# wangtong627/COR

Hardware: AMD Instinct MI355X
Metric: query triplets/sec (forward + similarity + top-k) (higher is better)
Workload: dtype bf16

## Files before the change

cor_amd/_native.py:

```python
from __future__ import annotations

import ctypes as C
import os

_HERE = os.path.dirname(os.path.abspath(__file__))
LIB_PATH = os.environ.get("COR_AMD_LIB") or os.path.join(_HERE, "csrc", "libcor_amd.so")

F32, BF16, F16, BF16X3 = 0, 1, 2, 3
ACT_NONE, ACT_GELU_ERF, ACT_RELU, ACT_SIGMOID, ACT_GELU_TANH = 0, 1, 2, 3, 4
EINVAL, ENOSUPPORT = -1, -2
TOPK_FORCE_LISTS, TOPK_NO_FALLBACK, TOPK_FORCE_GLOBAL_THRESHOLD, TOPK_WAVE_FINAL = 1, 2, 8, 16
TOPK_KMAX = 256
FILTER_EQ, FILTER_NE = 0, 1
MERGE_NMAX = 4096
ORDER_REVERSE = 1 << 30
KERNEL_ROWLANE, KERNEL_FEWQ, KERNEL_FLASH_MFMA, KERNEL_FLASH_PIPELINED, KERNEL_WINDOW_BLOCK = 1, 2, 3, 4, 5
import numpy as _np
Q_PRESCALE_HD64 = float(_np.float32(0.125) * _np.float32(1.4426950408889634))

_p, _i, _l, _f, _ll = C.c_void_p, C.c_int, C.c_long, C.c_float, C.c_longlong

SIGNATURES = {
    "cor_version": [],
    "cor_gemm": [_p, _l, _p, _l, _i, _p, _l, _i, _i, _i, _i, _p, _i, _p, _p, _l, _i, _i, _p],
    "cor_layernorm": [_p, _i, _p, _i, _p, _p, _i, _i, _f, _i, _p],
    "cor_attention": [_p, _l, _l, _p, _l, _l, _p, _l, _l, _i, _p, _l, _l, _i, _i, _i, _i, _i, _i, _f, _p],
    "cor_attention_f32": [_p, _l, _l, _p, _l, _l, _p, _l, _l, _p, _l, _l, _i, _i, _i, _i, _i, _i, _f, _p],
    "cor_attention_kernel_id": [_i, _i, _i, _i, _i, _i],
    "cor_sam_attention": [_p, _i, _p, _i, _p, _p, _p, _i, _i, _i, _i, _i, _f, _i, _p],
    "cor_patchify": [_p, _p, _i, _i, _i, _i, _i, _i, _i, _p],
    "cor_im2col3x3": [_p, _i, _p, _i, _i, _i, _i, _p],
    "cor_add": [_p, _i, _p, _i, _p, _i, _l, _l, _p],
    "cor_copy_rows": [_p, _l, _i, _p, _l, _i, _i, _i, _p],
    "cor_split_x3": [_p, _l, _p, _l, _l, _i, _i, _p],
    "cor_tokens_to_nchw": [_p, _i, _p, _i, _i, _i, _p],
    "cor_nchw_to_tokens": [_p, _p, _i, _i, _i, _i, _p],
    "cor_l2norm_rows": [_p, _i, _p, _i, _i, _i, _f, _p],
    "cor_embed_tokens": [_p, _p, _p, _p, _i, _i, _i, _i, _p],
    "cor_bilinear": [_p, _p, _i, _i, _i, _i, _i, _i, _p],
    "cor_conv3x3s2_small": [_p, _i, _p, _p, _p, _i, _i, _i, _i, _i, _p],
    "cor_dwconv7x7": [_p, _p, _p, _p, _i, _i, _i, _i, _i, _p],
    "cor_adapter_pool": [_p, _p, _p, _i, _i, _i, _i, _p],
    "cor_masked_pool": [_p, _i, _p, _p, _i, _i, _i, _i, _i, _p],
    "cor_region_pool": [_p, _p, _p, _p, _i, _i, _i, _i, _i, _i, _i, _p],
    "cor_fuse_gate": [_p, _p, _p, _p, _p, _i, _i, _p],
    "cor_fuse_mix": [_p, _p, _p, _i, _i, _p],
    "cor_dense_pe": [_p, _p, _i, _i, _p],
    "cor_upscale_shuffle": [_p, _i, _p, _p, _p, _f, _i, _p, _i, _i, _i, _i, _i, _p],
# ... 63 lines not shown
```

cor_amd/csrc/flash_attn.hip:

```cpp
#include <cstdlib>
#include <type_traits>

#include "common.h"

typedef short s16x4 __attribute__((ext_vector_type(4)));

namespace {

struct FlashArgs {
  const bf16_t* q; const bf16_t* k; const bf16_t* v; void* o;
  long q_sb, q_st, k_sb, k_st, v_sb, v_st, o_sb, o_st;
  int H, Tq, Tk;
  float scale_log2;
  float tbl_scale;
  const bf16_t* pad_row; const float* rel_h; const float* rel_w;
  int grid, S, nW, d3;
  int nqt;
  int rev;
};

constexpr int KT = 64;
constexpr int TILE_B = KT * 128;
constexpr int KV_BYTES = 4 * TILE_B;
constexpr int AUX_PER_WAVE = 8192;
constexpr float LOG2E = 1.4426950408889634f;

__device__ __forceinline__ int acc_row(int e, int h) { return (e & 3) + 8 * (e >> 2) + 4 * h; }

__device__ __forceinline__ float other_half(float x) {
  const unsigned u = __float_as_uint(x);
  const auto r = __builtin_amdgcn_permlane32_swap(u, u, false, false);
  return __uint_as_float((threadIdx.x & 32) ? r[0] : r[1]);
}

typedef float f32x2_t __attribute__((ext_vector_type(2)));
typedef __bf16 bf16x2_t __attribute__((ext_vector_type(2)));
__device__ __forceinline__ uint32_t pk2(float a, float b) {
  const f32x2_t v = {a, b};
  return __builtin_bit_cast(uint32_t, __builtin_convertvector(v, bf16x2_t));
}
__device__ __forceinline__ uint4 pack8(float f0, float f1, float f2, float f3, float f4, float f5, float f6, float f7) {
  uint4 u;
  u.x = pk2(f0, f1); u.y = pk2(f2, f3); u.z = pk2(f4, f5); u.w = pk2(f6, f7);
  return u;
}

__device__ __forceinline__ float sum2_bf16(uint32_t pair, float acc) {
  return __builtin_amdgcn_fdot2_f32_bf16(__builtin_bit_cast(bf16x2_t, pair), __builtin_bit_cast(bf16x2_t, 0x3f803f80u), acc, false);
}
__device__ __forceinline__ float max3f_(float a, float b, float c) { return fmaxf(fmaxf(a, b), c); }

__device__ __forceinline__ uint4 table_frag(const float* tbl, int j, int c, int h) {
  const float* p = tbl + (long)j * 64 + 16 * c + 8 * h;
  const f32x4 a = *(const f32x4*)p, b = *(const f32x4*)(p + 4);
  return pack8(a[0], a[1], a[2], a[3], b[0], b[1], b[2], b[3]);
}

template <typename TO, int HD, typename OFF>
__device__ __forceinline__ void store_o_rows(const f32x16 (&o)[(HD + 31) / 32], float inv, char* stg, TO* out, int lane, OFF&& off) {
  constexpr int DB = (HD + 31) / 32;
  const int r = lane & 31, h = lane >> 5;
  if constexpr (sizeof(TO) == 2) {
    constexpr int SR = HD * 2 + 16, NCHO = HD * 2 / 16;
#pragma unroll
    for (int db = 0; db < DB; ++db)
#pragma unroll
      for (int g = 0; g < 4; ++g) {
        if (db * 32 + 8 * g + 8 <= HD) {
          uint2 u;
          u.x = pk2(o[db][4 * g] * inv, o[db][4 * g + 1] * inv); u.y = pk2(o[db][4 * g + 2] * inv, o[db][4 * g + 3] * inv);
          *(uint2*)(stg + r * SR + (db * 32 + 8 * g + 4 * h) * 2) = u;
        }
      }
    __builtin_amdgcn_fence(__ATOMIC_ACQ_REL, "wavefront");
#pragma unroll
    for (int i = 0; i < (32 * NCHO + 63) / 64; ++i) {
      const int idx = lane + 64 * i, j = idx / NCHO, ch = idx - j * NCHO;
      if (idx < 32 * NCHO) {
        const uint4 v = *(const uint4*)(stg + j * SR + ch * 16);
        const long e = off(j);
        if (e >= 0) *(uint4*)(out + e + ch * 8) = v;
      }
    }
// ... 929 lines not shown
    }
  }
  {
    asm volatile("s_waitcnt vmcnt(0)" ::: "memory");
    const char* Vs = Vring + ((nt - 1) & 3) * TILE_B;
#pragma unroll
    for (int kb = 0; kb < 2; ++kb)
#pragma unroll
      for (int ks = 0; ks < 2; ++ks)
#pragma unroll
        for (int db = 0; db < 2; ++db) {
          const char* vb = Vs + (kb * 32 + ks * 16) * 128 + v_trd[db];
          const s16x4 v0 = __builtin_amdgcn_ds_read_tr16_b64_v4i16((__attribute__((address_space(3))) s16x4*)(vb));
          const s16x4 v1 = __builtin_amdgcn_ds_read_tr16_b64_v4i16((__attribute__((address_space(3))) s16x4*)(vb + 8 * 128));
          const u32x4 vfr = __builtin_bit_cast(u32x4, __builtin_shufflevector(v0, v1, 0, 1, 2, 3, 4, 5, 6, 7));
#pragma unroll
          for (int qb = 0; qb < 2; ++qb)
            asm volatile("v_mfma_f32_32x32x16_bf16 %0, %1, %2, %0" : "+a"(o[qb][db]) : "a"(vfr), "v"(pf[qb][kb][ks]));
        }
    asm volatile("s_nop 7\n\ts_nop 7\n\ts_nop 7\n\ts_nop 7" ::: "memory");
  }
#pragma unroll
  for (int qb = 0; qb < 2; ++qb) {
    const float l = lsum[qb][0] + lsum[qb][1];
    const float inv = 1.0f / (l + other_half(l));
    auto off = [&](int j) -> long { return ((long)b * g2 + qh * S + qb * 32 + j) * (long)(a.H * 64) + head * 64; };
    store_o_rows<TO, 64>(o[qb], inv, (char*)aux, (TO*)a.o, lane, off);
    __builtin_amdgcn_fence(__ATOMIC_ACQ_REL, "wavefront");
  }
}

constexpr int WIN_ROWS = 224, WIN_KV = WIN_ROWS * 128, WIN_T = 27 * 32 * 4, WIN_LDS = 2 * WIN_KV + 7 * WIN_T;

template <typename TO>
__global__ void __launch_bounds__(448, 4) win_attn(const FlashArgs a) {
  extern __shared__ __attribute__((aligned(16))) char smem[];
  const int tid = threadIdx.x, lane = tid & 63, wave = __builtin_amdgcn_readfirstlane(tid >> 6);
  const int r = lane & 31, h = lane >> 5;
  const int bid = a.rev ? (int)gridDim.x - 1 - (int)blockIdx.x : (int)blockIdx.x;
  const int head = bid % a.H, win = bid / a.H;
  const int nw2 = a.nW * a.nW, b = win / nw2, wi = win - b * nw2, wy = wi / a.nW, wx = wi - wy * a.nW;
  const int g2 = a.grid * a.grid;
  char* Kt = smem; char* Vt = smem + WIN_KV;
  float* T = (float*)(smem + 2 * WIN_KV + wave * WIN_T);

  {
    const unsigned lds0 = __builtin_amdgcn_readfirstlane((unsigned)(size_t)((__attribute__((address_space(3))) char*)smem));
    const int sl = lane & 7;
    long colp[2]; bool okx[2];
#pragma unroll
    for (int hf = 0; hf < 2; ++hf) {
      const int kw = min(8 * hf + (lane >> 3), 13), x = wx * 14 + kw;
      okx[hf] = x < a.grid;
      colp[hf] = ((long)b * g2 + x) * a.d3 + head * 64;
    }
#pragma unroll
    for (int i8 = 0; i8 < 8; ++i8) {
      const int i = wave * 8 + i8;
      const bool isv = i >= 28;
      const int ii = isv ? i - 28 : i, kh = ii >> 1, hf = ii & 1, y = wy * 14 + kh;
      const int chunk = isv ? (sl ^ (((lane >> 4) & 1) << 2)) : (sl ^ (4 * hf + (lane >> 4)));
      const long plane = (long)(isv ? 2 : 1) * a.H * 64 + chunk * 8;
      const bf16_t* src = (y < a.grid && okx[hf]) ? a.q + colp[hf] + (long)y * a.grid * a.d3 + plane : a.pad_row + head * 64 + plane;
      glds16(src, lds0 + (isv ? WIN_KV : 0) + ii * 1024);
    }
  }

  const int tq = min(wave * 32 + r, 195);
  const int qh = (tq * 4682) >> 16, qw = tq - 14 * qh;
  uint4 qf[4];
  {
    const int y = wy * 14 + qh, x = wx * 14 + qw;
    const bf16_t* qp = (y < a.grid && x < a.grid) ? a.q + ((long)b * g2 + (long)y * a.grid + x) * a.d3 + head * 64 : a.pad_row + head * 64;
#pragma unroll
    for (int c = 0; c < 4; ++c) qf[c] = *(const uint4*)(qp + 16 * c + 8 * h);
  }

  float colb[8];
  uint4 tf[2][4];
#pragma unroll
  for (int tbl = 0; tbl < 2; ++tbl)
#pragma unroll
    for (int c = 0; c < 4; ++c) tf[tbl][c] = table_frag(tbl == 0 ? a.rel_w : a.rel_h, min(r, 26), c, h);
#pragma unroll
  for (int tbl = 0; tbl < 2; ++tbl) {
    f32x16 acc;
#pragma unroll
    for (int e = 0; e < 16; ++e) acc[e] = 0.f;
#pragma unroll
    for (int c = 0; c < 4; ++c)
      acc = __builtin_amdgcn_mfma_f32_32x32x16_bf16(__builtin_bit_cast(bf16x8, tf[tbl][c]), __builtin_bit_cast(bf16x8, qf[c]), acc, 0, 0, 0);
#pragma unroll
    for (int e = 0; e < 16; ++e) {
      const int row = acc_row(e, h);
      if (row < 27) T[row * 32 + r] = acc[e] * a.tbl_scale;
    }
    __builtin_amdgcn_fence(__ATOMIC_ACQ_REL, "wavefront");
    if (tbl == 0) {
#pragma unroll
      for (int e8 = 0; e8 < 8; ++e8) {
        const int kw = (e8 & 3) + 8 * (e8 >> 2) + 4 * h;
        colb[e8] = kw < 14 ? T[(qw - min(kw, 13) + 13) * 32 + r] : -INFINITY;
      }
      __builtin_amdgcn_fence(__ATOMIC_ACQ_REL, "wavefront");
    }
  }

  if (a.scale_log2 != 1.0f) {
#pragma unroll
    for (int c = 0; c < 4; ++c) {
      uint32_t w[4] = {qf[c].x, qf[c].y, qf[c].z, qf[c].w};
#pragma unroll
      for (int i = 0; i < 4; ++i) w[i] = pk2(__uint_as_float(w[i] << 16) * a.scale_log2, __uint_as_float(w[i] & 0xffff0000u) * a.scale_log2);
      qf[c] = make_uint4(w[0], w[1], w[2], w[3]);
    }
  }

  asm volatile("s_waitcnt vmcnt(0)" ::: "memory");
  __syncthreads();

  const int sw = (r >> 1) & 7;
  const int k_rd = r * 128, v_tr = (4 * h + ((lane & 15) >> 2)) * 128 + (16 * ((lane >> 4) & 1) + 4 * (lane & 3)) * 2;
  const int v_trd[2] = {v_tr + ((lane >> 3) & 1) * 64, v_tr + (1 - ((lane >> 3) & 1)) * 64};
  const int t_rd = (qh + 13) * 32 + r;
  f32x16 o[2], lsum;
#pragma unroll
  for (int e = 0; e < 16; ++e) { o[0][e] = 0.f; o[1][e] = 0.f; lsum[e] = 0.f; }
  float m = 0.f;
  const uint4 ones = make_uint4(0x3F803F80u, 0x3F803F80u, 0x3F803F80u, 0x3F803F80u);
#pragma unroll
  for (int blk = 0; blk < 7; ++blk) {
    const char* Kb = Kt + blk * 32 * 128 + k_rd;
    uint4 kf[4];
#pragma unroll
    for (int c = 0; c < 4; ++c) kf[c] = *(const uint4*)(Kb + (((2 * c + h) ^ sw) << 4));
    const float rm0 = T[t_rd - 32 * (2 * blk)] - m, rm1 = T[t_rd - 32 * (2 * blk + 1)] - m;
    f32x16 s;
#pragma unroll
    for (int e = 0; e < 16; ++e) s[e] = colb[e & 7] + (e < 8 ? rm0 : rm1);
#pragma unroll
    for (int c = 0; c < 4; ++c)
      s = __builtin_amdgcn_mfma_f32_32x32x16_bf16(__builtin_bit_cast(bf16x8, kf[c]), __builtin_bit_cast(bf16x8, qf[c]), s, 0, 0, 0);
    float mloc = max3f_(max3f_(s[0], s[1], s[2]), max3f_(s[3], s[4], s[5]), max3f_(s[6], s[7], s[8]));
    mloc = fmaxf(max3f_(mloc, max3f_(s[9], s[10], s[11]), max3f_(s[12], s[13], s[14])), s[15]);
    mloc = fmaxf(mloc, other_half(mloc));
    if (blk == 0 || __builtin_amdgcn_ballot_w64(mloc > 8.0f) != 0) {
      const float d = blk == 0 ? mloc : fmaxf(mloc, 0.f);
      const float alpha = __builtin_amdgcn_exp2f(-d);
      m += d;
#pragma unroll
      for (int e = 0; e < 16; ++e) s[e] -= d;
      if (blk != 0) {
        lsum[1] *= alpha; lsum[2] *= alpha;
#pragma unroll
        for (int e = 0; e < 16; ++e) { o[0][e] *= alpha; o[1][e] *= alpha; }
      }
    }
    uint4 pf[2];
    {
      f32x16 p;
#pragma unroll
      for (int e = 0; e < 16; ++e) p[e] = __builtin_amdgcn_exp2f(s[e]);
      pf[0] = pack8(p[0], p[1], p[2], p[3], p[4], p[5], p[6], p[7]);
      pf[1] = pack8(p[8], p[9], p[10], p[11], p[12], p[13], p[14], p[15]);
      lsum[1] = sum2_bf16(pf[0].y, sum2_bf16(pf[0].x, lsum[1])); lsum[2] = sum2_bf16(pf[0].w, sum2_bf16(pf[0].z, lsum[2]));
      lsum[1] = sum2_bf16(pf[1].y, sum2_bf16(pf[1].x, lsum[1])); lsum[2] = sum2_bf16(pf[1].w, sum2_bf16(pf[1].z, lsum[2]));
    }
#pragma unroll
    for (int ks = 0; ks < 2; ++ks) {
#pragma unroll
      for (int db = 0; db < 2; ++db) {
        const char* vb = Vt + (blk * 32 + ks * 16) * 128 + v_trd[db];
        const s16x4 v0 = __builtin_amdgcn_ds_read_tr16_b64_v4i16((__attribute__((address_space(3))) s16x4*)(vb));
        const s16x4 v1 = __builtin_amdgcn_ds_read_tr16_b64_v4i16((__attribute__((address_space(3))) s16x4*)(vb + 8 * 128));
        const uint2 u0 = __builtin_bit_cast(uint2, v0), u1 = __builtin_bit_cast(uint2, v1);
        const uint4 vfr = make_uint4(u0.x, u0.y, u1.x, u1.y);
        o[db] = __builtin_amdgcn_mfma_f32_32x32x16_bf16(__builtin_bit_cast(bf16x8, vfr), __builtin_bit_cast(bf16x8, pf[ks]), o[db], 0, 0, 0);
      }
    }
  }

  const float lhalf = lsum[1] + lsum[2];
  const float inv = 1.0f / (lhalf + other_half(lhalf));
  char* stg = (char*)T;
  TO* out = (TO*)a.o;
  auto off = [&](int jq) -> long {
    const int tj = wave * 32 + jq;
    if (tj >= 196) return -1;
    const int jh = (tj * 4682) >> 16, y = wy * 14 + jh, x = wx * 14 + (tj - 14 * jh);
    if (y >= a.grid || x >= a.grid) return -1;
    return ((long)b * g2 + (long)y * a.grid + x) * (long)(a.H * 64) + head * 64;
  };
  const long e0 = off(lane >> 2), e1 = off((lane >> 2) + 16);
  const int rd0 = (lane >> 2) * 80 + (lane & 3) * 16;
  __builtin_amdgcn_fence(__ATOMIC_ACQ_REL, "wavefront");
  if constexpr (sizeof(TO) == 2) {
#pragma unroll
    for (int db = 0; db < 2; ++db) {
#pragma unroll
      for (int g = 0; g < 4; ++g) {
        uint2 u;
        u.x = pk2(o[db][4 * g] * inv, o[db][4 * g + 1] * inv); u.y = pk2(o[db][4 * g + 2] * inv, o[db][4 * g + 3] * inv);
        *(uint2*)(stg + r * 80 + (8 * g + 4 * h) * 2) = u;
      }
      __builtin_amdgcn_fence(__ATOMIC_ACQ_REL, "wavefront");
      const uint4 v0 = *(const uint4*)(stg + rd0), v1 = *(const uint4*)(stg + rd0 + 16 * 80);
      if (e0 >= 0) *(uint4*)(out + e0 + db * 32 + (lane & 3) * 8) = v0;
      if (e1 >= 0) *(uint4*)(out + e1 + db * 32 + (lane & 3) * 8) = v1;
      __builtin_amdgcn_fence(__ATOMIC_ACQ_REL, "wavefront");
    }
  } else {
#pragma unroll
    for (int qd = 0; qd < 4; ++qd) {
      const int db = qd >> 1, g0 = 2 * (qd & 1);
#pragma unroll
      for (int gg = 0; gg < 2; ++gg) {
        const int g = g0 + gg;
        const f32x4 v4 = {o[db][4 * g] * inv, o[db][4 * g + 1] * inv, o[db][4 * g + 2] * inv, o[db][4 * g + 3] * inv};
        *(f32x4*)(stg + r * 80 + (8 * gg + 4 * h) * 4) = v4;
      }
      __builtin_amdgcn_fence(__ATOMIC_ACQ_REL, "wavefront");
      const f32x4 v0 = *(const f32x4*)(stg + rd0), v1 = *(const f32x4*)(stg + rd0 + 16 * 80);
      if (e0 >= 0) *(f32x4*)(out + e0 + qd * 16 + (lane & 3) * 4) = v0;
      if (e1 >= 0) *(f32x4*)(out + e1 + qd * 16 + (lane & 3) * 4) = v1;
      __builtin_amdgcn_fence(__ATOMIC_ACQ_REL, "wavefront");
    }
  }
}

template <typename TO>
int launch_win(const FlashArgs& a, int nwin, hipStream_t s) {
  static DevOnce once;
  cor_max_dyn_lds((const void*)win_attn<TO>, WIN_LDS, once);
  hipLaunchKernelGGL((win_attn<TO>), dim3(nwin * a.H), dim3(448), WIN_LDS, s, a);
  COR_CHECK_LAUNCH();
  return 0;
}

template <typename TO, bool STAMP = false, bool CB = false>
int launch_global_pipe(const FlashArgs& a, int nb, hipStream_t s) {
  const size_t lds = 6 * TILE_B + 4 * AUX_PER_WAVE;
  static DevOnce once;
  cor_max_dyn_lds((const void*)flash_global_pipe<TO, STAMP, CB>, (int)lds, once);
  FlashArgs b = a;
  b.nqt = cdiv(a.Tq, 128);
  hipLaunchKernelGGL((flash_global_pipe<TO, STAMP, CB>), dim3(b.nqt * a.H * nb), dim3(256), lds, s, b);
  COR_CHECK_LAUNCH();
  return 0;
}

template <typename TO, int DBG = 0>
int launch_global_w64(const FlashArgs& a, int nb, hipStream_t s) {
  const size_t lds = 8 * TILE_B + 4 * 64 * 64 * 4;
  static DevOnce once;
  cor_max_dyn_lds((const void*)flash_global_w64<TO, DBG>, (int)lds, once);
  FlashArgs b = a;
  b.nqt = a.Tq / 256;
  hipLaunchKernelGGL((flash_global_w64<TO, DBG>), dim3(b.nqt * a.H * nb), dim3(256), lds, s, b);
  COR_CHECK_LAUNCH();
  return 0;
}

template <int MODE, typename TO, int HD = 64>
int launch(const FlashArgs& a, int nb, hipStream_t s) {
  constexpr int ROWB = HD == 64 ? 128 : 208;
  const size_t lds = 4 * KT * ROWB + (MODE == 0 ? 0 : 4 * AUX_PER_WAVE);
  static DevOnce once;
// ... 2 lines not shown
  b.nqt = cdiv(a.Tq, 128);
  hipLaunchKernelGGL((flash_fwd<MODE, TO, HD>), dim3(b.nqt * a.H * nb), dim3(256), lds, s, b);
  COR_CHECK_LAUNCH();
  return 0;
}
template <int MODE, int HD>
int launch_t(const FlashArgs& a, int nb, int out_dtype, hipStream_t s) {
  if (out_dtype == COR_BF16) return launch<MODE, bf16_t, HD>(a, nb, s);
  if (out_dtype == COR_F32) return launch<MODE, float, HD>(a, nb, s);
  return COR_ENOSUPPORT;
}

}

int cor_flash_plain_bf16(const void* q, long q_sb, long q_st, const void* k, long k_sb, long k_st, const void* v, long v_sb, long v_st,
                         void* out, long o_sb, long o_st, int out_dtype, int B, int H, int Tq, int Tk, int hd, float scale, hipStream_t s) {
  if ((q_st | k_st | v_st | q_sb | k_sb | v_sb) & 7) return COR_ENOSUPPORT;
  if (((uintptr_t)q | (uintptr_t)k | (uintptr_t)v | (uintptr_t)out) & 15) return COR_ENOSUPPORT;
  if ((o_st | o_sb) & 7) return COR_ENOSUPPORT;
  FlashArgs a{};
  a.q = (const bf16_t*)q; a.k = (const bf16_t*)k; a.v = (const bf16_t*)v; a.o = out;
  a.q_sb = q_sb; a.q_st = q_st; a.k_sb = k_sb; a.k_st = k_st; a.v_sb = v_sb; a.v_st = v_st; a.o_sb = o_sb; a.o_st = o_st;
  a.H = H; a.Tq = Tq; a.Tk = Tk; a.scale_log2 = scale * LOG2E; a.tbl_scale = LOG2E; a.S = 1; a.grid = 1; a.nW = 1;
  if (hd == 64) return launch_t<0, 64>(a, B, out_dtype, s);
  if (hd == 72) return launch_t<0, 72>(a, B, out_dtype, s);
  if (hd == 80) return launch_t<0, 80>(a, B, out_dtype, s);
  return COR_ENOSUPPORT;
}

int cor_flash_sam_bf16(const void* qkv, void* out, int out_dtype, const void* pad_row, const float* rel_h, const float* rel_w, int B,
                       int H, int hd, int grid, int window, float q_prescale, int variant, hipStream_t s) {
  if (hd != 64 && hd != 80) return COR_ENOSUPPORT;
  const int rev = (variant & COR_ORDER_REVERSE) ? 1 : 0;
  variant &= ~COR_ORDER_REVERSE;
#ifdef COR_PROBES
  if (variant != 0 && variant != 1 && variant != 2 && variant != 4 && variant != 9 && !(variant >= 16 && variant < 4096)) return COR_EINVAL;
#else
  if (variant != 0 && variant != 1 && variant != 2 && variant != 4) return COR_EINVAL;
#endif
  if (((uintptr_t)qkv & 15) || ((uintptr_t)out & 15) || ((uintptr_t)rel_h & 15) || ((uintptr_t)rel_w & 15)) return COR_ENOSUPPORT;
  FlashArgs a{};
  a.q = (const bf16_t*)qkv; a.o = out; a.H = H; a.rev = rev;
  a.scale_log2 = LOG2E / sqrtf((float)hd) / q_prescale; a.tbl_scale = LOG2E / q_prescale;
  if (hd == 64 && fabsf(a.scale_log2 - 1.0f) < 1e-6f) { a.scale_log2 = 1.0f; a.tbl_scale = 8.0f; }
  a.pad_row = (const bf16_t*)pad_row; a.rel_h = rel_h; a.rel_w = rel_w; a.grid = grid; a.d3 = 3 * H * hd;
  if (window == 0) {
    if (grid != 64) return COR_ENOSUPPORT;
    a.S = 64; a.Tq = a.Tk = grid * grid; a.nW = 1;
#ifdef COR_PROBES
    if (const char* e = getenv("COR_ATTN_TK")) a.Tk = atoi(e);
#endif
    if (hd == 80) return launch_t<1, 80>(a, B, out_dtype, s);
#ifdef COR_PROBES
    if (variant >= 16 && out_dtype == COR_BF16 && a.scale_log2 == 1.0f) {
      switch (variant - 16) {
        case 1: return launch_global_w64<bf16_t, 1>(a, B, s);
        case 2: return launch_global_w64<bf16_t, 2>(a, B, s);
        case 3: return launch_global_w64<bf16_t, 3>(a, B, s);
        case 4: return launch_global_w64<bf16_t, 4>(a, B, s);
        case 8: return launch_global_w64<bf16_t, 8>(a, B, s);
        case 16: return launch_global_w64<bf16_t, 16>(a, B, s);
        case 32: return launch_global_w64<bf16_t, 32>(a, B, s);
        case 64: return launch_global_w64<bf16_t, 64>(a, B, s);
        case 96: return launch_global_w64<bf16_t, 96>(a, B, s);
        case 7: return launch_global_w64<bf16_t, 7>(a, B, s);
        case 127: return launch_global_w64<bf16_t, 127>(a, B, s);
        case 128: return launch_global_w64<bf16_t, 128>(a, B, s);
        case 256: return launch_global_w64<bf16_t, 256>(a, B, s);
        case 384: return launch_global_w64<bf16_t, 384>(a, B, s);
        case 512: return launch_global_w64<bf16_t, 512>(a, B, s);
        default: return COR_EINVAL;
      }
    }
    if (variant == 9) {
      if (out_dtype == COR_BF16) return launch_global_pipe<bf16_t, true>(a, B, s);
      if (out_dtype == COR_F32) return launch_global_pipe<float, true>(a, B, s);
    }
#endif
    if (variant == 4 && a.scale_log2 == 1.0f) {
      if (out_dtype == COR_BF16) return launch_global_w64<bf16_t>(a, B, s);
      if (out_dtype == COR_F32) return launch_global_w64<float>(a, B, s);
    }
    if (variant == 0 && a.scale_log2 == 1.0f) {
      if (out_dtype == COR_BF16) return launch_global_pipe<bf16_t, false, true>(a, B, s);
      if (out_dtype == COR_F32) return launch_global_pipe<float, false, true>(a, B, s);
    }
    if (variant == 0 || variant == 2 || variant == 4) {
      if (out_dtype == COR_BF16) return launch_global_pipe<bf16_t>(a, B, s);
      if (out_dtype == COR_F32) return launch_global_pipe<float>(a, B, s);
    }
    if (out_dtype == COR_BF16) return launch<1, bf16_t>(a, B, s);
    if (out_dtype == COR_F32) return launch<1, float>(a, B, s);
    return COR_ENOSUPPORT;
  }
  if (window != 14 || ((uintptr_t)pad_row & 15)) return COR_ENOSUPPORT;
  a.S = 14; a.Tq = a.Tk = 196; a.nW = (grid + 13) / 14;
  if (hd == 80) return launch_t<2, 80>(a, B * a.nW * a.nW, out_dtype, s);
  if (variant != 1) {
    if (out_dtype == COR_BF16) return launch_win<bf16_t>(a, B * a.nW * a.nW, s);
    if (out_dtype == COR_F32) return launch_win<float>(a, B * a.nW * a.nW, s);
    return COR_ENOSUPPORT;
  }
  if (out_dtype == COR_BF16) return launch<2, bf16_t>(a, B * a.nW * a.nW, s);
  if (out_dtype == COR_F32) return launch<2, float>(a, B * a.nW * a.nW, s);
  return COR_ENOSUPPORT;
}
```

cor_amd/engine.py:

```python
from __future__ import annotations

import math

import torch

from . import _native as nat
from . import ops
from .ops import ACT_NONE, ACT_GELU_ERF, ACT_RELU, ACT_SIGMOID, ACT_GELU_TANH, X3

F32 = torch.float32


def _round_up(x, m):
    return (x + m - 1) // m * m


class _Packer:

    def __init__(self, sd: dict, T: torch.dtype):
        dev = next(iter(sd.values())).device
        if dev.type != "cuda":
            raise RuntimeError("cor_amd: the model must live on a GPU (model.to('cuda')); there is no CPU path")
        self.sd, self.T, self.W = sd, T, {}

# ... 7 lines not shown
    def lin(self, p):
        self.mat(p + "weight")
        self.f32(p + "bias")

    def ln(self, p):
        self.f32(p + "weight")
        self.f32(p + "bias")

    def patch_embed(self, p, dim, patch):
        kp = 3 * patch * patch
        K = _round_up(kp, 16)
        self.W[p + "patch.K"] = K
        w = self.sd[p + "patch_embed.proj.weight"].detach().reshape(dim, kp)
        if K != kp:
            w = torch.nn.functional.pad(w, (0, K - kp))
        self.mat(p + "patch_embed.proj.weight", w)
        self.f32(p + "patch_embed.proj.bias")
        self.f32(p + "pos_embed", self.sd[p + "pos_embed"].detach().reshape(-1, dim))


def pack_sam_encoder(pk: _Packer, cfg: dict, p="image_encoder."):
    sd, W, d = pk.sd, pk.W, cfg["dim"]
    pk.patch_embed(p, d, cfg["patch"])
    for i in range(cfg["depth"]):
        b = f"{p}blocks.{i}."
        pk.ln(b + "norm1."); pk.ln(b + "norm2.")
        qs = nat.Q_PRESCALE_HD64 if (pk.T == torch.bfloat16 and d // cfg["heads"] == 64) else 1.0
        W[b + "attn.q_prescale"] = qs
        wq, bq = sd[b + "attn.qkv.weight"].detach().to(F32).clone(), sd[b + "attn.qkv.bias"].detach().to(F32).clone()
        wq[:d] *= qs; bq[:d] *= qs
        pk.mat(b + "attn.qkv.weight", wq); pk.f32(b + "attn.qkv.bias", bq)
        pk.lin(b + "attn.proj."); pk.lin(b + "mlp.lin1."); pk.lin(b + "mlp.lin2.")
        pk.f32(b + "attn.rel_pos_h"); pk.f32(b + "attn.rel_pos_w")
        pk.mat(b + "attn.pad_row", bq)
    pk.mat(p + "neck.0.weight", sd[p + "neck.0.weight"].detach().reshape(cfg["out"], d))
    pk.ln(p + "neck.1."); pk.ln(p + "neck.3.")
    w3 = sd[p + "neck.2.weight"].detach()
    pk.mat(p + "neck.2.weight", w3.permute(0, 2, 3, 1).reshape(w3.shape[0], -1))


def pack_prompt_encoder(pk: _Packer, p="prompt_encoder.", size=64):
    g = pk.sd[p + "pe_layer.positional_encoding_gaussian_matrix"].detach().to(F32).contiguous()
    pk.W["prompt.dense_pe"] = ops.dense_pe(g, size)
    pk.f32("prompt.no_mask", pk.sd[p + "no_mask_embed.weight"].detach().reshape(-1))


def pack_siglip(pk: _Packer, g: dict, p="support_branch.siglip.model."):
    v = p + "visual.trunk."
    pk.patch_embed(v, g["dim"], g["patch"])
    for i in range(g["depth"]):
        b = f"{v}blocks.{i}."
        pk.ln(b + "norm1."); pk.ln(b + "norm2.")
        pk.lin(b + "attn.qkv."); pk.lin(b + "attn.proj."); pk.lin(b + "mlp.fc1."); pk.lin(b + "mlp.fc2.")
    pk.ln(v + "norm.")
    t = p + "text."
    pk.f32(t + "token_embedding.weight"); pk.f32(t + "positional_embedding")
    for i in range(g["t_depth"]):
        b = f"{t}transformer.resblocks.{i}."
        pk.ln(b + "ln_1."); pk.ln(b + "ln_2.")
        pk.mat(b + "attn.in_proj_weight"); pk.f32(b + "attn.in_proj_bias")
        pk.lin(b + "attn.out_proj."); pk.lin(b + "mlp.c_fc."); pk.lin(b + "mlp.c_proj.")
    pk.ln(t + "ln_final."); pk.lin(t + "text_projection.")


def pack_mask_adapter(pk: _Packer, m="support_branch.mask_pooling."):
    sd = pk.sd
# ... 71 lines not shown
    pack_support_head(pkq, mask_pooling)
    pack_mask_decoder(pk)
    if pkq is not pk:
        pk.W.update(pkq.W)
    return pk.W


def _lin(W, p, a, out_dtype, act=ACT_NONE, residual=None, col_scale=None, out=None, reverse=False, x3=False):
    return ops.gemm(a, W[p + "weight"], out_dtype=out_dtype, bias=W[p + "bias"], act=act, residual=residual,
                    col_scale=col_scale, out=out, reverse=reverse, x3=x3)


def _ln(W, p, x, eps, out_dtype, act=ACT_NONE, reverse=False):
    return ops.layernorm(x, W[p + "weight"], W[p + "bias"], eps, out_dtype=out_dtype, act=act, reverse=reverse)


def _gelu(kind):
    return ACT_GELU_ERF if kind == "erf" else ACT_GELU_TANH


def sam_encoder(W, img, cfg, T, p="image_encoder."):
    B = img.shape[0]
    g, d, H = cfg["img"] // cfg["patch"], cfg["dim"], cfg["heads"]
    assert img.shape[1:] == (3, cfg["img"], cfg["img"]), f"SAM input must be [B,3,{cfg['img']},{cfg['img']}], got {tuple(img.shape)}"
    cols = ops.patchify(img, cfg["patch"], W[p + "patch.K"], T)
    x = ops.gemm(cols, W[p + "patch_embed.proj.weight"], out_dtype=F32, bias=W[p + "patch_embed.proj.bias"],
                 residual=W[p + "pos_embed"], res_row_mod=g * g)
    del cols
    for i in range(cfg["depth"]):
        b = f"{p}blocks.{i}."
        win = 0 if i in cfg["global_idx"] else cfg["window"]
        h = _ln(W, b + "norm1.", x, 1e-6, T, reverse=True)
        qkv = _lin(W, b + "attn.qkv.", h, T)
        a = ops.sam_attention(qkv, W[b + "attn.pad_row"], W[b + "attn.rel_pos_h"], W[b + "attn.rel_pos_w"], B, H, g, win,
                              q_prescale=W[b + "attn.q_prescale"], reverse=True)
        del qkv
        _lin(W, b + "attn.proj.", a, F32, residual=x, out=x)
        h = _ln(W, b + "norm2.", x, 1e-6, T, reverse=True)
        m = _lin(W, b + "mlp.lin1.", h, T, act=ACT_GELU_ERF)
        _lin(W, b + "mlp.lin2.", m, F32, residual=x, out=x)
        del h, a, m
    y = ops.gemm(ops.cast(x, T), W[p + "neck.0.weight"], out_dtype=F32)
    y = _ln(W, p + "neck.1.", y, 1e-6, T)
    y = ops.gemm(ops.im2col3x3(y, B, g, g), W[p + "neck.2.weight"], out_dtype=F32)
    return _ln(W, p + "neck.3.", y, 1e-6, F32)


def _vit_mha(qkv, N, Tn, heads, D, T):
    hd = D // heads
    if T == X3:
        return ops.attention_f32(qkv[:, 0:D], qkv[:, D:2 * D], qkv[:, 2 * D:3 * D], N, heads, Tn, Tn, hd, hd ** -0.5, out_dtype=X3)
    return ops.attention(qkv[:, 0:D], qkv[:, D:2 * D], qkv[:, 2 * D:3 * D], N, heads, Tn, Tn, hd, hd ** -0.5, out_dtype=T)


def _qkv_dtype(T):
    return F32 if T == X3 else T


def siglip_vision(W, img, g, T, p="support_branch.siglip.model.visual.trunk."):
    N = img.shape[0]
    D, P = g["dim"], (g["image"] // g["patch"]) ** 2
    x3 = T == X3
    assert img.shape[1:] == (3, g["image"], g["image"]), f"SigLIP input must be [N,3,{g['image']},{g['image']}], got {tuple(img.shape)}"
    cols = ops.patchify(img, g["patch"], W[p + "patch.K"], T)
    x = ops.gemm(cols, W[p + "patch_embed.proj.weight"], out_dtype=F32, bias=W[p + "patch_embed.proj.bias"],
                 residual=W[p + "pos_embed"], res_row_mod=P, x3=x3)
    act = _gelu(g.get("v_gelu", g.get("gelu", "erf")))
# ... 249 lines not shown
```

cor_amd/ops.py:

```python
from __future__ import annotations

import torch

from . import _native as nat
from ._native import ACT_NONE, ACT_GELU_ERF, ACT_RELU, ACT_SIGMOID, ACT_GELU_TANH, F32, BF16, F16

_DT = {torch.float32: F32, torch.bfloat16: BF16, torch.float16: F16}

X3 = "bf16x3"

GEMM_PROFILE = None


def _lib():
    return nat.load()


def _dt(t: torch.Tensor) -> int:
    return _DT[t.dtype]


def _s():
    return torch.cuda.current_stream().cuda_stream

# ... 100 lines not shown
    for t, T in ((q, Tq), (k, Tk), (v, Tk)):
        assert t.dim() == 2 and t.stride(1) == 1 and t.shape[0] == B * T and t.shape[1] == H * hd, (t.shape, B, T, H, hd)
    out = torch.empty((B * Tq, H * hd), dtype=out_dtype or q.dtype, device=q.device)
    nat.check(_lib().cor_attention(q.data_ptr(), Tq * q.stride(0), q.stride(0), k.data_ptr(), Tk * k.stride(0), k.stride(0),
                                   v.data_ptr(), Tk * v.stride(0), v.stride(0), _dt(q), out.data_ptr(), Tq * H * hd, H * hd,
                                   _dt(out), B, H, Tq, Tk, hd, float(scale), _s()), "cor_attention")
    return out


def attention_f32(q, k, v, B, H, Tq, Tk, hd, scale, out_dtype=torch.float32):
    _dev(q, k, v)
    for t, T in ((q, Tq), (k, Tk), (v, Tk)):
        assert t.dtype == torch.float32 and t.dim() == 2 and t.stride(1) == 1 and t.shape[0] == B * T and t.shape[1] == H * hd, (t.shape, B, T, H, hd)
    if out_dtype == X3:
        out = torch.empty((B * Tq, 3 * H * hd), dtype=torch.bfloat16, device=q.device)
        o_dt = nat.BF16X3
    else:
        assert out_dtype == torch.float32
        out = torch.empty((B * Tq, H * hd), dtype=torch.float32, device=q.device)
        o_dt = F32
    ld = out.shape[1]
    nat.check(_lib().cor_attention_f32(q.data_ptr(), Tq * q.stride(0), q.stride(0), k.data_ptr(), Tk * k.stride(0), k.stride(0),
                                       v.data_ptr(), Tk * v.stride(0), v.stride(0), out.data_ptr(), Tq * ld, ld, o_dt,
                                       B, H, Tq, Tk, hd, float(scale), _s()), "cor_attention_f32")
    return out


def sam_attention(qkv, pad_row, rel_h, rel_w, B, H, grid, window, out_dtype=None, variant=0, q_prescale=1.0, reverse=False):
    _dev(qkv, pad_row, rel_h, rel_w)
    hd = rel_h.shape[1]
    d = H * hd
    assert qkv.is_contiguous() and qkv.shape == (B * grid * grid, 3 * d), qkv.shape
    S = window if window > 0 else grid
    for r in (rel_h, rel_w):
        assert r.dtype == torch.float32 and r.is_contiguous() and r.shape == (2 * S - 1, hd), r.shape
    if window > 0:
        assert pad_row is not None and pad_row.dtype == qkv.dtype and pad_row.is_contiguous() and pad_row.numel() == 3 * d
    out = torch.empty((B * grid * grid, d), dtype=out_dtype or qkv.dtype, device=qkv.device)
    nat.check(_lib().cor_sam_attention(qkv.data_ptr(), _dt(qkv), out.data_ptr(), _dt(out), _p(pad_row), rel_h.data_ptr(),
                                       rel_w.data_ptr(), B, H, hd, grid, window, float(q_prescale), int(variant) | (nat.ORDER_REVERSE if reverse else 0), _s()), "cor_sam_attention")
    return out


def patchify(img, p, Kpad, out_dtype):
    if out_dtype == X3:
        return split_x3(patchify(img, p, Kpad, torch.float32))
    _dev(img)
    assert img.dtype == torch.float32 and img.is_contiguous() and img.dim() == 4
    B, C, H, W = img.shape
    out = torch.empty((B * (H // p) * (W // p), Kpad), dtype=out_dtype, device=img.device)
    nat.check(_lib().cor_patchify(img.data_ptr(), out.data_ptr(), _dt(out), B, C, H, W, p, Kpad, _s()), "cor_patchify")
    return out


def im2col3x3(x, B, H, W):
    _dev(x)
    C = x.shape[-1]
    assert x.is_contiguous() and x.numel() == B * H * W * C
    out = torch.empty((B * H * W, 9 * C), dtype=x.dtype, device=x.device)
    nat.check(_lib().cor_im2col3x3(x.data_ptr(), _dt(x), out.data_ptr(), B, H, W, C, _s()), "cor_im2col3x3")
    return out


def add(a, b, out_dtype=None, out=None):
    _dev(a, b, out)
    assert a.is_contiguous() and b.is_contiguous() and a.numel() % b.numel() == 0
    if out is None:
        out = torch.empty(a.shape, dtype=out_dtype or a.dtype, device=a.device)
    assert out.is_contiguous() and out.numel() == a.numel()
    nat.check(_lib().cor_add(a.data_ptr(), _dt(a), b.data_ptr(), _dt(b), out.data_ptr(), _dt(out), a.numel(), b.numel(), _s()),
              "cor_add")
    return out


# ... 385 lines not shown
```

include/cor_amd.h:

```cpp
#ifndef COR_AMD_H
#define COR_AMD_H

#ifdef __cplusplus
extern "C" {
#endif

#define COR_EINVAL (-1)
#define COR_ENOSUPPORT (-2)
#define COR_ORDER_REVERSE (1 << 30)
#define COR_TOPK_FORCE_LISTS 1
#define COR_TOPK_NO_FALLBACK 2
#define COR_TOPK_FORCE_GLOBAL_THRESHOLD 8
#define COR_TOPK_WAVE_FINAL 16
#define COR_TOPK_KMAX 256
#define COR_MERGE_NMAX 4096
#define COR_FILTER_EQ 0
#define COR_FILTER_NE 1

enum { COR_F32 = 0, COR_BF16 = 1, COR_F16 = 2 , COR_BF16X3 = 3  };
enum { COR_ACT_NONE = 0, COR_ACT_GELU_ERF = 1, COR_ACT_RELU = 2, COR_ACT_SIGMOID = 3, COR_ACT_GELU_TANH = 4 };

int cor_version(void);


int cor_gemm(const void* A, long lda, const void* W, long ldw, int ab_dtype,
             void* C, long ldc, int c_dtype, int M, int N, int K,
             const float* bias, int act, const float* col_scale,
             const float* residual, long ldr, int res_row_mod, int cfg, void* stream);

int cor_layernorm(const void* x, int x_dtype, void* y, int y_dtype, const float* w, const float* b,
                  int rows, int C, float eps, int act, void* stream);


int cor_attention(const void* q, long q_sb, long q_st, const void* k, long k_sb, long k_st,
                  const void* v, long v_sb, long v_st, int dtype,
                  void* out, long o_sb, long o_st, int out_dtype,
                  int B, int H, int Tq, int Tk, int hd, float scale, void* stream);

int cor_attention_f32(const float* q, long q_sb, long q_st, const float* k, long k_sb, long k_st,
                      const float* v, long v_sb, long v_st, void* out, long o_sb, long o_st, int out_dtype,
                      int B, int H, int Tq, int Tk, int hd, float scale, void* stream);

// ... 100 lines not shown
```

Before: 776.5.

## Streamline windowed SAM attention index math, KV staging, and bf16 rel-pos tables

Adds a new default form of the windowed attention kernel. It replaces integer div/mod with precomputed magic-multiply reciprocals and restructures the K/V global-to-LDS staging to use row-based addressing. It reduces across half-waves with a single permlane swap and computes output token offsets once per row, sharing them through LDS. Window-14 layers can also read relative-position tables pre-packed to bf16 at load time, which removes the per-launch fp32-to-bf16 packing but adds bf16 rounding of the tables and a new host-side weight path. Optional cycle-counter stamping is included for probe builds only.

```diff
diff --git a/cor_amd/_native.py b/cor_amd/_native.py
--- a/cor_amd/_native.py
+++ b/cor_amd/_native.py
@@ -14,6 +14,7 @@
 FILTER_EQ, FILTER_NE = 0, 1
 MERGE_NMAX = 4096
 ORDER_REVERSE = 1 << 30
+TABLES_BF16 = 1 << 29
 KERNEL_ROWLANE, KERNEL_FEWQ, KERNEL_FLASH_MFMA, KERNEL_FLASH_PIPELINED, KERNEL_WINDOW_BLOCK = 1, 2, 3, 4, 5
 import numpy as _np
 Q_PRESCALE_HD64 = float(_np.float32(0.125) * _np.float32(1.4426950408889634))
diff --git a/cor_amd/csrc/flash_attn.hip b/cor_amd/csrc/flash_attn.hip
--- a/cor_amd/csrc/flash_attn.hip
+++ b/cor_amd/csrc/flash_attn.hip
@@ -17,6 +17,8 @@
   int grid, S, nW, d3;
   int nqt;
   int rev;
+  int tbl_bf16;
+  unsigned mH, mW2, mW;
 };
 
 constexpr int KT = 64;
@@ -49,6 +51,16 @@
   return __builtin_amdgcn_fdot2_f32_bf16(__builtin_bit_cast(bf16x2_t, pair), __builtin_bit_cast(bf16x2_t, 0x3f803f80u), acc, false);
 }
 __device__ __forceinline__ float max3f_(float a, float b, float c) { return fmaxf(fmaxf(a, b), c); }
+__device__ __forceinline__ float both_halves_max(float x) {
+  const unsigned u = __float_as_uint(x);
+  const auto r = __builtin_amdgcn_permlane32_swap(u, u, false, false);
+  return fmaxf(__uint_as_float(r[0]), __uint_as_float(r[1]));
+}
+__device__ __forceinline__ float both_halves_sum(float x) {
+  const unsigned u = __float_as_uint(x);
+  const auto r = __builtin_amdgcn_permlane32_swap(u, u, false, false);
+  return __uint_as_float(r[0]) + __uint_as_float(r[1]);
+}
 
 __device__ __forceinline__ uint4 table_frag(const float* tbl, int j, int c, int h) {
   const float* p = tbl + (long)j * 64 + 16 * c + 8 * h;
@@ -1044,19 +1056,54 @@
 
 constexpr int WIN_ROWS = 224, WIN_KV = WIN_ROWS * 128, WIN_T = 27 * 32 * 4, WIN_LDS = 2 * WIN_KV + 7 * WIN_T;
 
-template <typename TO>
+template <typename TO, int FORM = 1, bool STAMP = false>
 __global__ void __launch_bounds__(448, 4) win_attn(const FlashArgs a) {
   extern __shared__ __attribute__((aligned(16))) char smem[];
   const int tid = threadIdx.x, lane = tid & 63, wave = __builtin_amdgcn_readfirstlane(tid >> 6);
   const int r = lane & 31, h = lane >> 5;
+  unsigned long long ts[6];
+  auto stamp = [&](int i) { if (STAMP) { __builtin_amdgcn_sched_barrier(0); ts[i] = __builtin_readcyclecounter(); __builtin_amdgcn_sched_barrier(0); } };
+  stamp(0);
   const int bid = a.rev ? (int)gridDim.x - 1 - (int)blockIdx.x : (int)blockIdx.x;
-  const int head = bid % a.H, win = bid / a.H;
-  const int nw2 = a.nW * a.nW, b = win / nw2, wi = win - b * nw2, wy = wi / a.nW, wx = wi - wy * a.nW;
+  int head, win, b, wi, wy, wx;
+  const int nw2 = a.nW * a.nW;
+  if constexpr (FORM == 0) {
+    head = bid % a.H; win = bid / a.H;
+    b = win / nw2; wi = win - b * nw2; wy = wi / a.nW; wx = wi - wy * a.nW;
+  } else {
+    win = (int)__umulhi((unsigned)bid << 1, a.mH); head = bid - win * a.H;
+    b = (int)__umulhi((unsigned)win << 1, a.mW2); wi = win - b * nw2;
+    wy = (int)__umulhi((unsigned)wi << 1, a.mW); wx = wi - wy * a.nW;
+  }
   const int g2 = a.grid * a.grid;
   char* Kt = smem; char* Vt = smem + WIN_KV;
   float* T = (float*)(smem + 2 * WIN_KV + wave * WIN_T);
 
-  {
+  if constexpr (FORM != 0) {
+    const unsigned lds0 = __builtin_amdgcn_readfirstlane((unsigned)(size_t)((__attribute__((address_space(3))) char*)smem));
+    const int sl = lane & 7, y0 = wy * 14 + 2 * wave;
+    const long rowstride = (long)a.grid * a.d3;
+    const bf16_t* qrow = a.q + ((long)b * g2 + (long)y0 * a.grid) * a.d3 + head * 64;
+    const bf16_t* padh = a.pad_row + head * 64;
+    int xo[2]; bool okx[2];
+#pragma unroll
+    for (int hf = 0; hf < 2; ++hf) {
+      const int kw = min(8 * hf + (lane >> 3), 13), x = wx * 14 + kw;
+      okx[hf] = x < a.grid;
+      xo[hf] = x * a.d3;
+    }
+#pragma unroll
+    for (int isv = 0; isv < 2; ++isv)
+#pragma unroll
+      for (int rr = 0; rr < 2; ++rr)
+#pragma unroll
+        for (int hf = 0; hf < 2; ++hf) {
+          const int chunk = isv ? (sl ^ (((lane >> 4) & 1) << 2)) : (sl ^ (4 * hf + (lane >> 4)));
+          const int eoff = (isv ? 2 : 1) * a.H * 64 + chunk * 8;
+          const bf16_t* src = (y0 + rr < a.grid && okx[hf]) ? qrow + rr * rowstride + xo[hf] + eoff : padh + eoff;
+          glds16(src, lds0 + (isv ? WIN_KV : 0) + (4 * wave + 2 * rr + hf) * 1024);
+        }
+  } else {
     const unsigned lds0 = __builtin_amdgcn_readfirstlane((unsigned)(size_t)((__attribute__((address_space(3))) char*)smem));
     const int sl = lane & 7;
     long colp[2]; bool okx[2];
@@ -1081,19 +1128,26 @@
   const int tq = min(wave * 32 + r, 195);
   const int qh = (tq * 4682) >> 16, qw = tq - 14 * qh;
   uint4 qf[4];
+  int tok = -1;
   {
     const int y = wy * 14 + qh, x = wx * 14 + qw;
     const bf16_t* qp = (y < a.grid && x < a.grid) ? a.q + ((long)b * g2 + (long)y * a.grid + x) * a.d3 + head * 64 : a.pad_row + head * 64;
 #pragma unroll
     for (int c = 0; c < 4; ++c) qf[c] = *(const uint4*)(qp + 16 * c + 8 * h);
-  }
+    if constexpr (FORM != 0) tok = (wave * 32 + r < 196 && y < a.grid && x < a.grid) ? b * g2 + y * a.grid + x : -1;
+  }
+  stamp(1);
 
   float colb[8];
   uint4 tf[2][4];
 #pragma unroll
   for (int tbl = 0; tbl < 2; ++tbl)
 #pragma unroll
-    for (int c = 0; c < 4; ++c) tf[tbl][c] = table_frag(tbl == 0 ? a.rel_w : a.rel_h, min(r, 26), c, h);
+    for (int c = 0; c < 4; ++c) {
+      const float* tb = tbl == 0 ? a.rel_w : a.rel_h;
+      if (FORM != 0 && a.tbl_bf16) tf[tbl][c] = *(const uint4*)((const bf16_t*)tb + min(r, 26) * 64 + 16 * c + 8 * h);
+      else tf[tbl][c] = table_frag(tb, min(r, 26), c, h);
+    }
 #pragma unroll
   for (int tbl = 0; tbl < 2; ++tbl) {
     f32x16 acc;
@@ -1128,8 +1182,10 @@
     }
   }
 
+  stamp(2);
   asm volatile("s_waitcnt vmcnt(0)" ::: "memory");
   __syncthreads();
+  stamp(3);
 
   const int sw = (r >> 1) & 7;
   const int k_rd = r * 128, v_tr = (4 * h + ((lane & 15) >> 2)) * 128 + (16 * ((lane >> 4) & 1) + 4 * (lane & 3)) * 2;
@@ -1155,7 +1211,8 @@
       s = __builtin_amdgcn_mfma_f32_32x32x16_bf16(__builtin_bit_cast(bf16x8, kf[c]), __builtin_bit_cast(bf16x8, qf[c]), s, 0, 0, 0);
     float mloc = max3f_(max3f_(s[0], s[1], s[2]), max3f_(s[3], s[4], s[5]), max3f_(s[6], s[7], s[8]));
     mloc = fmaxf(max3f_(mloc, max3f_(s[9], s[10], s[11]), max3f_(s[12], s[13], s[14])), s[15]);
-    mloc = fmaxf(mloc, other_half(mloc));
+    if constexpr (FORM == 0) mloc = fmaxf(mloc, other_half(mloc));
+    else mloc = both_halves_max(mloc);
     if (blk == 0 || __builtin_amdgcn_ballot_w64(mloc > 8.0f) != 0) {
       const float d = blk == 0 ? mloc : fmaxf(mloc, 0.f);
       const float alpha = __builtin_amdgcn_exp2f(-d);
@@ -1192,8 +1249,9 @@
     }
   }
 
+  stamp(4);
   const float lhalf = lsum[1] + lsum[2];
-  const float inv = 1.0f / (lhalf + other_half(lhalf));
+  const float inv = 1.0f / (FORM == 0 ? lhalf + other_half(lhalf) : both_halves_sum(lhalf));
   char* stg = (char*)T;
   TO* out = (TO*)a.o;
   auto off = [&](int jq) -> long {
@@ -1203,7 +1261,18 @@
     if (y >= a.grid || x >= a.grid) return -1;
     return ((long)b * g2 + (long)y * a.grid + x) * (long)(a.H * 64) + head * 64;
   };
-  const long e0 = off(lane >> 2), e1 = off((lane >> 2) + 16);
+  long e0, e1;
+  if constexpr (FORM == 0) {
+    e0 = off(lane >> 2); e1 = off((lane >> 2) + 16);
+  } else {
+    int* tk = (int*)(stg + 2560);
+    __builtin_amdgcn_fence(__ATOMIC_ACQ_REL, "wavefront");
+    tk[r] = tok;
+    __builtin_amdgcn_fence(__ATOMIC_ACQ_REL, "wavefront");
+    const int t0 = tk[lane >> 2], t1 = tk[(lane >> 2) + 16];
+    e0 = t0 < 0 ? -1L : (long)t0 * (long)(a.H * 64) + head * 64;
+    e1 = t1 < 0 ? -1L : (long)t1 * (long)(a.H * 64) + head * 64;
+  }
   const int rd0 = (lane >> 2) * 80 + (lane & 3) * 16;
   __builtin_amdgcn_fence(__ATOMIC_ACQ_REL, "wavefront");
   if constexpr (sizeof(TO) == 2) {
@@ -1238,13 +1307,23 @@
       __builtin_amdgcn_fence(__ATOMIC_ACQ_REL, "wavefront");
     }
   }
-}
-
-template <typename TO>
+  if (STAMP) {
+    asm volatile("s_waitcnt vmcnt(0)" ::: "memory");
+    stamp(5);
+    if (lane == 0)
+#pragma unroll
+      for (int i = 0; i < 5; ++i) ((unsigned long long*)a.o)[((long)blockIdx.x * 7 + wave) * 8 + i] = ts[i + 1] - ts[i];
+  }
+}
+
+template <typename TO, int FORM = 1, bool STAMP = false>
 int launch_win(const FlashArgs& a, int nwin, hipStream_t s) {
   static DevOnce once;
-  cor_max_dyn_lds((const void*)win_attn<TO>, WIN_LDS, once);
-  hipLaunchKernelGGL((win_attn<TO>), dim3(nwin * a.H), dim3(448), WIN_LDS, s, a);
+  cor_max_dyn_lds((const void*)win_attn<TO, FORM, STAMP>, WIN_LDS, once);
+  FlashArgs w = a;
+  const int nw2 = a.nW * a.nW;
+  w.mH = (1u << 31) / (unsigned)a.H + 1; w.mW2 = (1u << 31) / (unsigned)nw2 + 1; w.mW = (1u << 31) / (unsigned)a.nW + 1;
+  hipLaunchKernelGGL((win_attn<TO, FORM, STAMP>), dim3(nwin * a.H), dim3(448), WIN_LDS, s, w);
   COR_CHECK_LAUNCH();
   return 0;
 }
@@ -1313,12 +1392,14 @@
                        int H, int hd, int grid, int window, float q_prescale, int variant, hipStream_t s) {
   if (hd != 64 && hd != 80) return COR_ENOSUPPORT;
   const int rev = (variant & COR_ORDER_REVERSE) ? 1 : 0;
-  variant &= ~COR_ORDER_REVERSE;
+  const int tbl_bf16 = (variant & COR_TABLES_BF16) ? 1 : 0;
+  variant &= ~(COR_ORDER_REVERSE | COR_TABLES_BF16);
 #ifdef COR_PROBES
-  if (variant != 0 && variant != 1 && variant != 2 && variant != 4 && variant != 9 && !(variant >= 16 && variant < 4096)) return COR_EINVAL;
+  if (variant != 0 && variant != 1 && variant != 2 && variant != 4 && variant != 7 && variant != 9 && variant != 11 && !(variant >= 16 && variant < 4096)) return COR_EINVAL;
 #else
-  if (variant != 0 && variant != 1 && variant != 2 && variant != 4) return COR_EINVAL;
+  if (variant != 0 && variant != 1 && variant != 2 && variant != 4 && variant != 7) return COR_EINVAL;
 #endif
+  if (tbl_bf16 && !(window == 14 && hd == 64 && variant == 0)) return COR_EINVAL;
   if (((uintptr_t)qkv & 15) || ((uintptr_t)out & 15) || ((uintptr_t)rel_h & 15) || ((uintptr_t)rel_w & 15)) return COR_ENOSUPPORT;
   FlashArgs a{};
   a.q = (const bf16_t*)qkv; a.o = out; a.H = H; a.rev = rev;
@@ -1328,6 +1409,7 @@
   if (window == 0) {
     if (grid != 64) return COR_ENOSUPPORT;
     a.S = 64; a.Tq = a.Tk = grid * grid; a.nW = 1;
+    if (variant == 7 || variant == 11) return COR_EINVAL;
 #ifdef COR_PROBES
     if (const char* e = getenv("COR_ATTN_TK")) a.Tk = atoi(e);
 #endif
@@ -1378,8 +1460,23 @@
   a.S = 14; a.Tq = a.Tk = 196; a.nW = (grid + 13) / 14;
   if (hd == 80) return launch_t<2, 80>(a, B * a.nW * a.nW, out_dtype, s);
   if (variant != 1) {
-    if (out_dtype == COR_BF16) return launch_win<bf16_t>(a, B * a.nW * a.nW, s);
-    if (out_dtype == COR_F32) return launch_win<float>(a, B * a.nW * a.nW, s);
+    const int nwin = B * a.nW * a.nW;
+    a.tbl_bf16 = tbl_bf16;
+    const bool small = (long)nwin * H * (H > a.nW * a.nW ? H : a.nW * a.nW) < (1L << 31) && (long)B * grid * grid < (1L << 31);
+#ifdef COR_PROBES
+    if (variant == 9 || variant == 11) {
+      if (!small || (long)a.nW * a.nW * 448 > (long)grid * grid * 128 || out_dtype != COR_BF16) return COR_EINVAL;
+      return variant == 9 ? launch_win<bf16_t, 1, true>(a, nwin, s) : launch_win<bf16_t, 0, true>(a, nwin, s);
+    }
+#endif
+    if (variant == 7 || !small) {
+      if (tbl_bf16) return COR_ENOSUPPORT;
+      if (out_dtype == COR_BF16) return launch_win<bf16_t, 0>(a, nwin, s);
+      if (out_dtype == COR_F32) return launch_win<float, 0>(a, nwin, s);
+      return COR_ENOSUPPORT;
+    }
+    if (out_dtype == COR_BF16) return launch_win<bf16_t, 1>(a, nwin, s);
+    if (out_dtype == COR_F32) return launch_win<float, 1>(a, nwin, s);
     return COR_ENOSUPPORT;
   }
   if (out_dtype == COR_BF16) return launch<2, bf16_t>(a, B * a.nW * a.nW, s);
diff --git a/cor_amd/engine.py b/cor_amd/engine.py
--- a/cor_amd/engine.py
+++ b/cor_amd/engine.py
@@ -63,6 +63,8 @@
         pk.mat(b + "attn.qkv.weight", wq); pk.f32(b + "attn.qkv.bias", bq)
         pk.lin(b + "attn.proj."); pk.lin(b + "mlp.lin1."); pk.lin(b + "mlp.lin2.")
         pk.f32(b + "attn.rel_pos_h"); pk.f32(b + "attn.rel_pos_w")
+        if qs != 1.0 and i not in cfg["global_idx"] and cfg["window"] == 14:
+            W[b + "attn.rel_pos_h.bf16"], W[b + "attn.rel_pos_w.bf16"] = ops.pack_rel_tables(W[b + "attn.rel_pos_h"], W[b + "attn.rel_pos_w"])
         pk.mat(b + "attn.pad_row", bq)
     pk.mat(p + "neck.0.weight", sd[p + "neck.0.weight"].detach().reshape(cfg["out"], d))
     pk.ln(p + "neck.1."); pk.ln(p + "neck.3.")
@@ -200,7 +202,8 @@
         win = 0 if i in cfg["global_idx"] else cfg["window"]
         h = _ln(W, b + "norm1.", x, 1e-6, T, reverse=True)
         qkv = _lin(W, b + "attn.qkv.", h, T)
-        a = ops.sam_attention(qkv, W[b + "attn.pad_row"], W[b + "attn.rel_pos_h"], W[b + "attn.rel_pos_w"], B, H, g, win,
+        rk = ".bf16" if (b + "attn.rel_pos_h.bf16") in W and win == 14 else ""
+        a = ops.sam_attention(qkv, W[b + "attn.pad_row"], W[b + "attn.rel_pos_h" + rk], W[b + "attn.rel_pos_w" + rk], B, H, g, win,
                               q_prescale=W[b + "attn.q_prescale"], reverse=True)
         del qkv
         _lin(W, b + "attn.proj.", a, F32, residual=x, out=x)
diff --git a/cor_amd/ops.py b/cor_amd/ops.py
--- a/cor_amd/ops.py
+++ b/cor_amd/ops.py
@@ -156,14 +156,19 @@
     d = H * hd
     assert qkv.is_contiguous() and qkv.shape == (B * grid * grid, 3 * d), qkv.shape
     S = window if window > 0 else grid
+    packed = rel_h.dtype == torch.bfloat16
     for r in (rel_h, rel_w):
-        assert r.dtype == torch.float32 and r.is_contiguous() and r.shape == (2 * S - 1, hd), r.shape
+        assert r.dtype == (torch.bfloat16 if packed else torch.float32) and r.is_contiguous() and r.shape == (2 * S - 1, hd), r.shape
     if window > 0:
         assert pad_row is not None and pad_row.dtype == qkv.dtype and pad_row.is_contiguous() and pad_row.numel() == 3 * d
     out = torch.empty((B * grid * grid, d), dtype=out_dtype or qkv.dtype, device=qkv.device)
     nat.check(_lib().cor_sam_attention(qkv.data_ptr(), _dt(qkv), out.data_ptr(), _dt(out), _p(pad_row), rel_h.data_ptr(),
-                                       rel_w.data_ptr(), B, H, hd, grid, window, float(q_prescale), int(variant) | (nat.ORDER_REVERSE if reverse else 0), _s()), "cor_sam_attention")
-    return out
+                                       rel_w.data_ptr(), B, H, hd, grid, window, float(q_prescale), int(variant) | (nat.ORDER_REVERSE if reverse else 0) | (nat.TABLES_BF16 if packed else 0), _s()), "cor_sam_attention")
+    return out
+
+
+def pack_rel_tables(rel_h, rel_w):
+    return rel_h.to(torch.bfloat16).contiguous(), rel_w.to(torch.bfloat16).contiguous()
 
 
 def patchify(img, p, Kpad, out_dtype):
diff --git a/include/cor_amd.h b/include/cor_amd.h
--- a/include/cor_amd.h
+++ b/include/cor_amd.h
@@ -8,6 +8,7 @@
 #define COR_EINVAL (-1)
 #define COR_ENOSUPPORT (-2)
 #define COR_ORDER_REVERSE (1 << 30)
+#define COR_TABLES_BF16 (1 << 29)
 #define COR_TOPK_FORCE_LISTS 1
 #define COR_TOPK_NO_FALLBACK 2
 #define COR_TOPK_FORCE_GLOBAL_THRESHOLD 8
```

Result: no change. 780.3 (median of 6 runs) (+0.5%).
